# RegulatoryGenomicsGroup/chicdiff

Hardware: AMD Instinct MI355X
Metric: interactions/sec NB-GLM Wald test (higher is better)
Workload: dtype f64; 1 GPU; synthetic 2000000 interactions x 8 samples (4v4), size factors + offsets(theta=0.5) + dispersions + Wald, design ~condition; rows_per_gpu=2000000, samples=8, global_rows=2000000, parallelism=rows-sharded x1, collectives=none (single rank), ranks_in_communicator=1

## Files before the change

### chicdiff_amd/csrc/common.h

```cpp
#pragma once
#include <hip/hip_runtime.h>
#include <stdint.h>

#include "../../include/chicdiff_hip.h"
#include "fit_driver.h"
#include "fit_state.h"

namespace cd {

constexpr int kRedBlocks = 1024;

struct FitDims {
    int64_t n;
    int32_t S, p, nA, nB;
    uint64_t gmask;
};

struct FitWork {
    double *baseMean, *baseVar, *gm0, *gm1, *rough, *binit0, *binit1, *crow;
    double *dispGene, *dispFit, *dispMAP, *disp, *beta0, *beta1, *resid;
    int32_t *allZero, *geneIter, *mapIter, *outlier, *betaIter, *optimConv;
    int32_t *order;
    uint8_t *cls;
    int32_t *gridlist;
// ... 27 lines not shown
    return chunk > first_back && (uint32_t)old < stop_f;
}
__host__ __device__ inline uint32_t filler_stop_f(int percent, uint32_t chunks, uint32_t first_back) {
    if (percent >= 100) return 0xffffffffu;
    if (percent <= 0) return 0u;
    const uint32_t own = first_back < chunks ? first_back : chunks;
    return (uint32_t)(((unsigned long long)own * (unsigned)percent + 99ull) / 100ull);
}
constexpr int kRowHdr = 32;
__host__ __device__ inline int64_t row_stride(int S) {
    const int64_t bytes = kRowHdr + (int64_t)S * 12;
    return bytes <= 64 ? 64 : (bytes + 127) / 128 * 128;
}
__device__ __forceinline__ double *row_hdr(char *rowpack, int64_t r, int S) { return reinterpret_cast<double *>(rowpack + r * row_stride(S)); }

struct Opts {
    double minDisp, dispTol, kappa0, betaTol, minmu, outlierSD, dispPriorVarIn, maxDisp, trendIn[2];
    int32_t maxit, betaMaxit;
    int32_t fit_type = 0;
    int32_t spread = 1;
    int32_t min_waves = 0;
    int32_t schedule = 1;
    int32_t deal = 0;
    int32_t chunk = 0;
    int32_t classes_a = 0;
    int32_t xim_here = 0;
    int32_t prio = 0;
    int32_t fillers = -1;
    int32_t filler_stop = -1;
    int32_t trend_blocks = 0;
    int32_t trend_speculate = 1;
    int32_t mad_route = 1;
    int32_t mad_value_cap = 0;
};

constexpr int kSchedClasses = 6, kSchedBlocks = 1024;
inline void order_tiles(int64_t n, int64_t &nblk, int64_t &tile) {
    nblk = (n + 255) / 256;
    if (nblk > kSchedBlocks) nblk = kSchedBlocks;
    tile = ((n + nblk - 1) / nblk + 255) / 256 * 256;
    nblk = (n + tile - 1) / tile;
}
constexpr int kSchedClassesFine = 23, kSchedEdgesFine = 21, kSchedMinDispSlot = 17;
constexpr int kSchedSix = 3, kSchedMinDispLast = 4;
__host__ __device__ inline int sched_class(double a0, double gmin, double minDisp, int mode) {
    constexpr double edge[kSchedEdgesFine] = {0.0316, 0.0422, 0.0562, 0.0750, 0.1, 0.1334, 0.1778, 0.2371, 0.316, 0.4217, 0.5623,
                                              0.7499, 1.0, 1.3335, 1.7783, 2.3714, 3.16, 4.2170, 5.6234, 7.4989, 10.0};
    if (!(a0 > 1.5 * minDisp)) return (mode == kSchedSix || mode == kSchedMinDispLast) ? kSchedClassesFine - 1 : kSchedMinDispSlot;
    const double s = a0 * gmin;
    int f = 0;
    if (mode == kSchedSix) {
#pragma unroll
        for (int k = 4; k < kSchedEdgesFine; k += 4) f += !(s < edge[k]) ? 4 : 0;
        f += f > 0 ? 1 : 0;
    } else {
#pragma unroll
        for (int k = 0; k < kSchedEdgesFine; k++) f += !(s < edge[k]) ? 1 : 0;
    }
    return f < kSchedMinDispSlot ? f : f + 1;
}
__host__ __device__ inline int sched_classes_a(int a, int mode) {
    if (a <= 0) return 0;
    if (a <= 3) return 1 + 4 * a;
    if (a == 4) return kSchedMinDispSlot;
    if (a == 5) return (mode == kSchedSix || mode == kSchedMinDispLast) ? kSchedClassesFine - 1 : kSchedMinDispSlot;
    return kSchedClassesFine;
// ... 264 lines not shown
```

### chicdiff_amd/csrc/ctx.hip

```cpp
#include <stdarg.h>

#include <dlfcn.h>

#include "ctx.h"

char cd::g_create_err[512];

const PmcTable &cd::pmc_table(int df) {
    static PmcTable tables[4];
    static bool ready[4] = {false, false, false, false};
    static std::mutex mu;
    std::lock_guard<std::mutex> lock(mu);
    if (!ready[df]) {
        pmc_build(df, tables[df]);
        ready[df] = true;
    }
    return tables[df];
}

int cd::fail(chicdiff_hip_ctx *c, int code, const char *fmt, ...) {
    va_list ap;
    va_start(ap, fmt);
    vsnprintf(c ? c->err : g_create_err, 512, fmt, ap);
    va_end(ap);
// ... 24 lines not shown
    int32_t Opts::*tune;
    int HostOpts::*host;
    int64_t lo, hi, no_lo, no_hi;
};
static const OptionDef kOptions[] = {
    {"line_search_spread", &Opts::spread, nullptr, 0, 3, 1, 0},
    {"line_search_min_waves", &Opts::min_waves, nullptr, 0, 4, 1, 1},
    {"line_search_chunk", &Opts::chunk, nullptr, 0, 64, 1, 7},
    {"line_search_prio", &Opts::prio, nullptr, 0, 100, 1, 0},
    {"line_search_schedule", &Opts::schedule, nullptr, 0, 4, 2, 2},
    {"line_search_deal", &Opts::deal, nullptr, 0, 64, 1, 0},
    {"line_search_classes_a", &Opts::classes_a, nullptr, 0, 6, 1, 0},
    {"line_search_fillers", &Opts::fillers, nullptr, -1, 1, 1, 0},
    {"line_search_filler_stop", &Opts::filler_stop, nullptr, -1, 100, 1, 0},
    {"theta_grid_concurrency", nullptr, &HostOpts::theta_grid_concurrency, 1, 16, 1, 0},
    {"host_copy_threads", nullptr, &HostOpts::host_copy_threads, 1, 64, 1, 0},
    {"select_all_rounds", nullptr, &HostOpts::select_all_rounds, 0, 1, 1, 0},
    {"trend_one_launch_per_pass", nullptr, &HostOpts::trend_one_launch_per_pass, 0, 1, 1, 0},
    {"sharded_trend_gather", nullptr, &HostOpts::sharded_trend_gather, 0, 1, 1, 0},
    {"trend_persistent_blocks", &Opts::trend_blocks, nullptr, 0, 256, 1, 0},
    {"trend_speculate", &Opts::trend_speculate, nullptr, 0, 1, 1, 0},
    {"mad_select_route", &Opts::mad_route, nullptr, 0, 1, 1, 0},
    {"mad_value_cap", &Opts::mad_value_cap, nullptr, 0, kVbCap, 1, 0},
    {"trend_mad_in_kernel", nullptr, &HostOpts::trend_mad_in_kernel, 0, 1, 1, 0},
    {"fuse_offsets", nullptr, &HostOpts::fuse_offsets, 0, 2, 1, 0},
    {"prep_blocks", nullptr, &HostOpts::prep_blocks, 0, kRedBlocks, 1, 0},
    {"region_assemble_generic", nullptr, &HostOpts::region_assemble_generic, 0, 1, 1, 0},
    {"chicago_tables_run_merge", nullptr, &HostOpts::chicago_tables_run_merge, 0, 1, 1, 0},
    {"table_write_half_kib", nullptr, &HostOpts::table_write_half_kib, 0, 65536, 1, 3},
    {"fault_inject", nullptr, &HostOpts::fault_inject, 0, 7, 1, 0},
    {"bench_fake_world", nullptr, &HostOpts::bench_fake_world, 0, kGatherMaxWorld, 1, 0},
    {"sf_log_table", nullptr, &HostOpts::sf_log_table, 0, 1, 1, 0},
    {"wald_final_row_constant", nullptr, &HostOpts::wald_final_row_constant, 0, 1, 1, 0},
    {"local_trend_substitute", nullptr, &HostOpts::local_trend_substitute, 0, 1, 1, 0},
};

int chicdiff_hip_set_option(chicdiff_hip_ctx *c, const char *name, int64_t value) {
    if (!c || !name) return CHICDIFF_E_INVALID;
    for (const OptionDef &d : kOptions) {
        if (strcmp(name, d.name) != 0 || value < d.lo || value > d.hi || (value >= d.no_lo && value <= d.no_hi)) continue;
        if (d.host == &HostOpts::bench_fake_world && value > 1 && !getenv("CHICDIFF_BENCH_FAKE_WORLD"))
            return fail(c, CHICDIFF_E_INVALID, "set_option: bench_fake_world is a rehearsal hook of bench.py (CHICDIFF_BENCH_FAKE_WORLD unset)");
        if (d.tune) c->tune.*d.tune = (int32_t)value;
        else c->host.*d.host = (int)value;
        return CHICDIFF_OK;
    }
    return fail(c, CHICDIFF_E_INVALID, "set_option: unknown option or value (%s = %lld)", name, (long long)value);
}

int chicdiff_hip_create(chicdiff_hip_ctx **out, int32_t device) {
    if (!out) return fail(nullptr, CHICDIFF_E_INVALID, "ctx out pointer is NULL");
    *out = nullptr;
    int ndev = 0;
    hipError_t e = hipGetDeviceCount(&ndev);
    if (e != hipSuccess || ndev <= 0)
        return fail(nullptr, CHICDIFF_E_HIP, "no HIP device available (%s): the HIP path cannot run, and there is no CPU fallback",
                    e != hipSuccess ? hipGetErrorString(e) : "device count 0");
    if (device < 0 || device >= ndev) return fail(nullptr, CHICDIFF_E_INVALID, "device %d out of range [0,%d)", device, ndev);
    chicdiff_hip_ctx *c = new chicdiff_hip_ctx();
    c->device = device;
    if ((e = hipSetDevice(device)) != hipSuccess || (e = hipStreamCreateWithFlags(&c->own_stream, hipStreamNonBlocking)) != hipSuccess ||
        (e = hipHostMalloc((void **)&c->h_sc, sizeof(FitScalars))) != hipSuccess ||
        (e = hipHostMalloc((void **)&c->h_sf, sizeof(double) * (kMaxS + 1))) != hipSuccess ||
        (e = hipMalloc((void **)&c->d_sf, sizeof(double) * (kMaxS + 1 + kSelMaxWorld + 8))) != hipSuccess ||
        (e = hipMemset(c->d_sf, 0, sizeof(double) * (kMaxS + 1 + kSelMaxWorld + 8))) != hipSuccess ||
        (e = hipMalloc((void **)&c->d_logfact, sizeof(double) * kLogFactN)) != hipSuccess) {
// ... 390 lines not shown
```

### chicdiff_amd/csrc/wald_kernels.hip

```cpp
#include "common.h"
#include "devmath.h"

namespace cd {

constexpr double kLog2e = 1.4426950408889634074;

__global__ __launch_bounds__(256) void wald_prep_kernel(const int32_t *__restrict__ counts,
                                                        const double *__restrict__ nf, FitDims d, FitWork w, int sched, int64_t tile, unsigned int *hist) {
    __shared__ double s_logfact[kLogFactN];
    __shared__ LogEntry s_lt[64];
    for (int k = threadIdx.x; k < kLogFactN; k += 256) s_logfact[k] = w.logfact[k];
    log_table_to_lds(s_lt);
    const int64_t n = d.n;
    const int S = d.S;
    unsigned int mine[kSchedClasses] = {0, 0, 0, 0, 0, 0};
    const int64_t lo = tile > 0 ? (int64_t)blockIdx.x * tile : (int64_t)blockIdx.x * 256;
    const int64_t hi = tile > 0 ? (lo + tile < n ? lo + tile : n) : n;
    const int64_t step = tile > 0 ? 256 : (int64_t)gridDim.x * 256;
    for (int64_t i = lo + threadIdx.x; i < hi; i += step) {
        if (w.allZero[i]) {
            reinterpret_cast<double2 *>(w.start)[2 * i] = make_double2(NAN, 0.0);
            if (sched) {
                w.cls[i] = 255;
                w.beta0[i] = NAN;
// ... 25 lines not shown
            if ((d.gmask >> j) & 1) lB += l; else lA += l;
            if (yi > 0) {
                c += lgr_eval_t(cs, yi, s_lt) - (yi < kLogFactN ? s_logfact[yi] : lgr_eval(c1, yi));
                cst = fma((double)yi, la + tlog(nfj, s_lt), cst);
            }
        }
        lA /= d.nA;
        lB /= d.nB;
        w.binit0[i] = lA;
        w.binit1[i] = lB - lA;
        w.crow[i] = c;
        double2 *h = reinterpret_cast<double2 *>(w.start) + 2 * i;
        h[0] = make_double2(alpha, c + cst);
        h[1] = make_double2(lA, lB - lA);
    }
    if (tile > 0) order_hist_store(mine, hist);
}


__device__ __forceinline__ double optim_objective(const int32_t *y_, const double *f_, int64_t stride, int S, uint64_t gmask,
                                                  double alpha, double size, double la, double crow, double lam, double b0,
                                                  double b1) {
    double f = 0.5 * lam * (b0 * b0 + b1 * b1) - crow;
    const double E0 = exp(b0), E1 = exp(b0 + b1);
    for (int j = 0; j < S; j++) {
        const double y = (double)y_[j * stride];
        const double mu = f_[j * stride] * (((gmask >> j) & 1) ? E1 : E0);
        const double ma = alpha * mu, t = 1.0 + ma;
        f += (size + y) * flog1p_from(ma, t, rcp(t));
        if (y > 0) f -= y * (la + flog(mu));
    }
    return f;
}
__device__ __noinline__ bool optim_row(const int32_t *y_, const double *f_, int64_t stride, int S, uint64_t gmask, double alpha, double crow,
                                       double &b0, double &b1) {
    const double lam = 1e-6 / (0.69314718055994530942 * 0.69314718055994530942);
    const double bound = 30.0 * 0.69314718055994530942;
    const double size = rcp(alpha), la = flog(alpha);
    double f = optim_objective(y_, f_, stride, S, gmask, alpha, size, la, crow, lam, b0, b1);
    bool converged = false;
    for (int it = 0; it < 200 && !converged; it++) {
        double g0 = lam * b0, g1 = lam * b1, wA = 0, wB = 0;
        const double E0 = exp(b0), E1 = exp(b0 + b1);
        for (int j = 0; j < S; j++) {
            const bool g = (gmask >> j) & 1;
            const double y = (double)y_[j * stride];
            const double mu = f_[j * stride] * (g ? E1 : E0);
            const double rt = rcp(fma(alpha, mu, 1.0));
            const double sc = (y - mu) * rt, wj = mu * rt;
            g0 -= sc;
            if (g) { g1 -= sc; wB += wj; } else wA += wj;
        }
        const double m00 = wA + wB + lam, m01 = wB, m11 = wB + lam, det = m00 * m11 - m01 * m01;
        const double d0 = -(m11 * g0 - m01 * g1) / det, d1 = -(m00 * g1 - m01 * g0) / det;
        double t = 1.0;
        bool moved = false;
        for (int h = 0; h < 40; h++, t *= 0.5) {
            const double n0 = fmin(fmax(b0 + t * d0, -bound), bound), n1 = fmin(fmax(b1 + t * d1, -bound), bound);
            const double fn = optim_objective(y_, f_, stride, S, gmask, alpha, size, la, crow, lam, n0, n1);
            if (fn < f) {
                if (f - fn < 1e-13 * (fabs(f) + 1.0)) converged = true;
                b0 = n0; b1 = n1; f = fn; moved = true;
                break;
            }
        }
        if (!moved) converged = true;
    }
// ... 36 lines not shown
    if (S == 4) return load_row_sums_fixed<1>(row, s_nf, s_y, lane, gmask, iyA, iyB);
    if (S == 16) return load_row_sums_fixed<4>(row, s_nf, s_y, lane, gmask, iyA, iyB);
    if (S == 12) return load_row_sums_fixed<3>(row, s_nf, s_y, lane, gmask, iyA, iyB);
    const double *pf = reinterpret_cast<const double *>(row + kRowHdr);
    const int *py = reinterpret_cast<const int *>(row + kRowHdr + 8 * S);
    int a = 0, b = 0;
    for (int j = 0; j < S; j++) {
        const int yi = py[j];
        s_nf[j * 64 + lane] = pf[j];
        s_y[j * 64 + lane] = yi;
        if ((gmask >> j) & 1) b += yi; else a += yi;
    }
    iyA = a;
    iyB = b;
}

#ifdef CHICDIFF_DIAG
#define WDIAG(...) __VA_ARGS__
__device__ unsigned long long g_irls_cy[8], g_irls_open[2];
#else
#define WDIAG(...)
#endif
struct WaldArgs {
    const int32_t *counts;
    const double *nf;
    FitDims d;
    FitWork w;
    Opts o;
    int chunk;
    const int32_t *order;
    int spread;
};

#ifndef WALD_MINW
#define WALD_MINW 3
#endif
__global__ __launch_bounds__(256, WALD_MINW) void wald_irls_kernel(WaldArgs A) {
    extern __shared__ double smem[];
    __shared__ LogEntry s_logtab[64];
    __shared__ ExpEntry s_exptab[64];
    exp_table_to_lds(s_exptab);
    log_table_to_lds(s_logtab);
    const int lane = threadIdx.x & 63;
    const int wave = __builtin_amdgcn_readfirstlane((int)(threadIdx.x >> 6));
    const int S = A.d.S;
    const int64_t n = A.d.n;
    double *s_nf = smem + (size_t)wave * S * 96;
    int *s_y = reinterpret_cast<int *>(s_nf + S * 64);
    const uint64_t gmask = A.d.gmask;
    const Opts o = A.o;
    const double lambda = 1e-6 / (0.69314718055994530942 * 0.69314718055994530942);
    const int32_t *__restrict__ order = A.order;
    const uint32_t nTot = order ? (uint32_t)A.w.sc->ord_n : (uint32_t)n;
    unsigned long long *heads = A.w.queue + 32;
    int cur_head = blockIdx.x & 7;
    unsigned int heads_left = 0xffu;
    const uint32_t nchunks = (nTot + (uint32_t)A.chunk - 1u) / (uint32_t)A.chunk;
    const int64_t rstride = row_stride(S);

    int spread_lg = A.spread ? 1 : -1;
    while (spread_lg >= 0 && (1 << spread_lg) < S) spread_lg++;

    bool need = true, done = false, queue_empty = false;
    uint32_t chunk_pos = 0, chunk_len = 0, rest_base = 0, rest_end = 0;
    int ord_reg = 0;
    int row = -1;
    int k = 0;
    double b0 = 0, b1 = 0, alpha = 0, size = 0, crow = 0, dev_old = 0, syA = 0, syB = 0;

    WDIAG(unsigned long long cyw[8] = {0, 0, 0, 0, 0, 0, 0, 0}, wt_eval_end = 0, wr_load_end = 0, g_open_cy = 0, g_open_n = 0;)
    for (;;) {
        WDIAG(const int sec = 0; const bool sec_bulk = !queue_empty; const unsigned long long wt0 = __builtin_amdgcn_s_memtime();)
        unsigned long long needmask = __ballot(need && !done);
#pragma unroll 1
        for (int attempt = 0; needmask != 0ull && attempt < 4; attempt++) {
            WDIAG(const unsigned long long wo0 = __builtin_amdgcn_s_memtime(); const bool opened = chunk_pos >= chunk_len;)
            if (chunk_pos >= chunk_len) {
                if (rest_base >= rest_end) {
                    if (queue_empty) {
                        if (need) done = true;
                        break;
                    }
                    if (heads_left == 0u) {
                        queue_empty = true;
                        continue;
                    }
                    unsigned int kq = 0;
                    if (lane == 0) kq = (unsigned int)atomicAdd(heads + 8 * cur_head, 1ull);
                    kq = __builtin_amdgcn_readfirstlane(kq);
                    const uint32_t cq = kq * 8u + (uint32_t)cur_head;
                    if (cq >= nchunks) {
                        heads_left &= ~(1u << cur_head);
                        for (int t = 1; t <= 8; t++) {
                            const int hn = (cur_head + t) & 7;
                            if (heads_left & (1u << hn)) { cur_head = hn; break; }
                        }
                        continue;
                    }
                    rest_base = cq * (uint32_t)A.chunk;
                    rest_end = rest_base + (uint32_t)A.chunk < nTot ? rest_base + (uint32_t)A.chunk : nTot;
                }
                const uint32_t b = rest_base;
                chunk_len = rest_end - rest_base < 64u ? rest_end - rest_base : 64u;
                rest_base += chunk_len;
                chunk_pos = 0;
                ord_reg = (int)b + lane;
                if (order && (uint32_t)lane < chunk_len) ord_reg = order[b + lane];
            }
            WDIAG(if (opened && !queue_empty) { g_open_cy += __builtin_amdgcn_s_memtime() - wo0; g_open_n++; })
            const uint32_t cnt = (uint32_t)__popcll(needmask), avail = chunk_len - chunk_pos;
            const uint32_t take = cnt < avail ? cnt : avail;
            const uint32_t rank = __builtin_amdgcn_mbcnt_hi((uint32_t)(needmask >> 32), __builtin_amdgcn_mbcnt_lo((uint32_t)needmask, 0u));
            const int r = __shfl(ord_reg, (int)((chunk_pos + rank) & 63u));
            chunk_pos += take;
            WDIAG(const unsigned long long wr0 = __builtin_amdgcn_s_memtime();)
            if (need && !done && rank < take) {
                int iyA = 0, iyB = 0;
                const double2 *stp = reinterpret_cast<const double2 *>(A.w.start) + 2 * (int64_t)r;
                const double2 st0 = stp[0], st1 = stp[1];
                load_row_sums(A.w.rowpack + (int64_t)r * rstride, S, s_nf, s_y, lane, gmask, iyA, iyB);
                WDIAG(const unsigned long long wr1 = __builtin_amdgcn_s_memtime(); if (!queue_empty) { cyw[4] += wr0 - wt0; cyw[5] += wr1 - wr0; cyw[7]++; } wr_load_end = wr1;)
                if (st0.x != st0.x) {
                    A.w.beta0[r] = NAN;
                    A.w.beta1[r] = NAN;
                    A.w.betaIter[r] = 0;
                } else {
                    row = r;
                    syA = (double)iyA;
                    syB = (double)iyB;
                    alpha = st0.x;
                    size = 1.0 / alpha;
                    crow = st0.y;
                    b0 = st1.x;
                    b1 = st1.y;
                    k = 0;
                    dev_old = 0;
                    need = false;
                }
            }
            needmask = __ballot(need && !done);
            WDIAG(if (wr_load_end) { if (!queue_empty) cyw[6] += __builtin_amdgcn_s_memtime() - wr_load_end; wr_load_end = 0; })
        }
        if (__ballot(!done) == 0ull) break;
        WDIAG(const unsigned long long wt1 = __builtin_amdgcn_s_memtime();)
        const bool active = !need && !done;
        const unsigned long long actmask = __ballot(active);
        double wA = 0, wB = 0, uA = 0, uB = 0, Dl = 0, zcA = 0, zcB = 0, Dc = 0;
        const bool spread_now = queue_empty && spread_lg >= 0 && (__popcll(actmask) << spread_lg) <= 64;
        if (spread_now) {
            const int grp = lane >> spread_lg, jj = lane & ((1 << spread_lg) - 1);
            int owner = 0, nact = 0;
            for (unsigned long long m = actmask; m; m &= m - 1ull, nact++)
                if (grp == nact) owner = __ffsll((long long)m) - 1;
            const bool mine = grp < nact && jj < S;
            const double b0o = __shfl(b0, owner), b1o = __shfl(b1, owner), alo = __shfl(alpha, owner), szo = __shfl(size, owner);
            const double etaAo = b0o, etaBo = b0o + b1o;
            const double E0 = texp(etaAo, s_exptab), E1 = texp(etaBo, s_exptab);
            const double nfj = mine ? s_nf[jj * 64 + owner] : 1.0;
            const double y = mine ? (double)s_y[jj * 64 + owner] : 0.0;
            const bool g = (gmask >> jj) & 1;
            const double raw = nfj * (g ? E1 : E0);
            const bool floored = raw < o.minmu;
            const double mu = floored ? o.minmu : raw;
            const double ma = alo * mu;
            const double t1 = 1.0 + ma;
            const double rt = rcp(t1);
            const double wj = mu * rt;
            const double yr = y * rt;
            const double sy = szo + y;
            const double L = tlog1p_from(ma, t1, rt, s_logtab);
            double de = 0.0;
            if (floored) de = (tlog(o.minmu, s_logtab) - tlog(nfj, s_logtab)) - (g ? etaBo : etaAo);
            const int fl = floored ? 1 : 0;
            const int base = grp << spread_lg;
            for (int j0 = 0; j0 < S; j0 += 4) {
                double q_wj[4], q_yr[4], q_sy[4], q_L[4], q_de[4], q_y[4];
                int q_fl[4];
#pragma unroll
                for (int t = 0; t < 4; t++) {
                    const int src = base + (j0 + t < S ? j0 + t : j0);
                    q_wj[t] = __shfl(wj, src);
                    q_yr[t] = __shfl(yr, src);
                    q_sy[t] = __shfl(sy, src);
                    q_L[t] = __shfl(L, src);
                    q_fl[t] = __shfl(fl, src);
                    q_de[t] = __shfl(de, src);
                    q_y[t] = __shfl(y, src);
                }
#pragma unroll
                for (int t = 0; t < 4; t++) {
                    if (j0 + t >= S) continue;
                    const bool gj = (gmask >> (j0 + t)) & 1;
                    const double gB = gj ? 1.0 : 0.0, gA = gj ? 0.0 : 1.0;
                    wA = fma(q_wj[t], gA, wA);
                    wB = fma(q_wj[t], gB, wB);
                    uA = fma(q_yr[t], gA, uA);
                    uB = fma(q_yr[t], gB, uB);
                    Dl = fma(q_sy[t], q_L[t], Dl);
                    if (q_fl[t]) {
                        if (gj) zcB = fma(q_wj[t], q_de[t], zcB); else zcA = fma(q_wj[t], q_de[t], zcA);
                        Dc = fma(-q_y[t], q_de[t], Dc);
                    }
                }
            }
            const int src = (active ? __popcll(actmask & ((1ull << lane) - 1ull)) : 0) << spread_lg;
            wA = __shfl(wA, src);
            wB = __shfl(wB, src);
            uA = __shfl(uA, src);
            uB = __shfl(uB, src);
            Dl = __shfl(Dl, src);
            zcA = __shfl(zcA, src);
            zcB = __shfl(zcB, src);
            Dc = __shfl(Dc, src);
        }
        if (active) {

            const double etaA = b0, etaB = b0 + b1;
            double E0 = 0, E1 = 0;
            if (!spread_now) {
                E0 = texp(etaA, s_exptab);
                E1 = texp(etaB, s_exptab);
            }
            for (int j = 0; j < (spread_now ? 0 : S); j++) {
                const double nfj = s_nf[j * 64 + lane];
                const double y = (double)s_y[j * 64 + lane];
                const bool g = (gmask >> j) & 1;
                const double raw = nfj * (g ? E1 : E0);
                const bool floored = raw < o.minmu;
                const double mu = floored ? o.minmu : raw;
                const double ma = alpha * mu;
                const double t1 = 1.0 + ma;
                const double rt = rcp(t1);
                const double wj = mu * rt;
                const double gB = g ? 1.0 : 0.0, gA = g ? 0.0 : 1.0;
                const double yr = y * rt;
                wA = fma(wj, gA, wA);
                wB = fma(wj, gB, wB);
                uA = fma(yr, gA, uA);
                uB = fma(yr, gB, uB);
                Dl = fma(size + y, tlog1p_from(ma, t1, rt, s_logtab), Dl);
                if (floored) {
                    const double de = (tlog(o.minmu, s_logtab) - tlog(nfj, s_logtab)) - (g ? etaB : etaA);
                    if (g) zcB = fma(wj, de, zcB); else zcA = fma(wj, de, zcA);
                    Dc = fma(-y, de, Dc);
                }
            }
            WDIAG(const unsigned long long wt2 = __builtin_amdgcn_s_memtime(); if (sec_bulk) { cyw[sec + 0] += wt1 - wt0; cyw[sec + 1] += wt2 - wt1; cyw[sec + 3]++; wt_eval_end = wt2; })
            const double zA = fma(etaA - 1.0, wA, uA) + zcA, zB = fma(etaB - 1.0, wB, uB) + zcB;
            const double D = (Dl - fma(etaA, syA, etaB * syB)) + Dc;
            bool stop = false;
            int iter_out = k;
            if (k >= 1) {
                const double dev = 2.0 * (D - crow);
                const double diff = fabs(dev - dev_old), scale = fabs(dev) + 0.1;
                if (!(diff == diff) || !(scale == scale) || (isinf(diff) && isinf(scale))) {
                    stop = true;
                    iter_out = o.betaMaxit;
                } else if (k >= 2 && diff < o.betaTol * scale) {
                    stop = true;
                } else if (k >= o.betaMaxit) {
                    stop = true;
                }
                dev_old = dev;
            }
            if (!stop) {
                const double m00 = wA + wB + lambda, m01 = wB, m11 = wB + lambda;
                const double r0 = zA + zB, r1 = zB;
                const double idet = rcp(fma(m00, m11, -(m01 * m01)));
                b0 = fma(m11, r0, -(m01 * r1)) * idet;
                b1 = fma(m00, r1, -(m01 * r0)) * idet;
                k++;
                if (fabs(b0) > 30.0 || fabs(b1) > 30.0) {
                    stop = true;
                    iter_out = o.betaMaxit;
                }
            }
            if (stop) {
                if (iter_out >= o.betaMaxit) {
                    b0 = A.w.binit0[row];
                    b1 = A.w.binit1[row];
                    A.w.optimConv[row] = optim_row(s_y + lane, s_nf + lane, 64, S, gmask, alpha, A.w.crow[row], b0, b1) ? 1 : 0;
                }
                A.w.beta0[row] = b0;
                A.w.beta1[row] = b1;
                A.w.betaIter[row] = iter_out;
                need = true;
            }
        }
        WDIAG(if (wt_eval_end) { cyw[sec + 2] += __builtin_amdgcn_s_memtime() - wt_eval_end; wt_eval_end = 0; })
    }
    WDIAG(if (lane == 0) { for (int q = 0; q < 8; q++) atomicAdd(&g_irls_cy[q], cyw[q]); atomicAdd(&g_irls_open[0], g_open_cy); atomicAdd(&g_irls_open[1], g_open_n); })
}


__device__ __forceinline__ int trim_lo(int n) {
    const double tr = n <= 3 ? 1.0 / 3 : (n <= 23 ? 1.0 / 4 : 1.0 / 8);
    return (int)floor(n * tr);
}
__device__ __forceinline__ double trim_scale(int n) { return n <= 3 ? 2.04 : (n <= 23 ? 1.86 : 1.51); }

__device__ __forceinline__ double cell_trimmed_mean(const double *s_q, int T, int tid, int S, uint64_t gmask, int c,
                                                    int nc, int lo, bool sq, double cm) {
    double sum = 0;
    if (lo == 1) {
        int imin = -1, imax = -1;
        double vmin = INFINITY, vmax = -INFINITY;
        for (int j = 0; j < S; j++) {
            if ((int)((gmask >> j) & 1) != c) continue;
            double vj = s_q[j * T + tid];
            if (sq) vj = (vj - cm) * (vj - cm);
            if (vj < vmin) { vmin = vj; imin = j; }
            if (vj >= vmax) { vmax = vj; imax = j; }
        }
        for (int j = 0; j < S; j++) {
            if ((int)((gmask >> j) & 1) != c || j == imin || j == imax) continue;
            double vj = s_q[j * T + tid];
            if (sq) vj = (vj - cm) * (vj - cm);
            sum += vj;
        }
        return sum / (nc - 2);
    }
    for (int j = 0; j < S; j++) {
// ... 243 lines not shown
        for (int b = threadIdx.x; b < kRedBlocks; b += 256) acc += w.partials[(size_t)b * 3 + k];
        red[threadIdx.x] = acc;
        __syncthreads();
        for (int s = 128; s > 0; s >>= 1) {
            if ((int)threadIdx.x < s) red[threadIdx.x] += red[threadIdx.x + s];
            __syncthreads();
        }
        if (threadIdx.x == 0) sums[k] = red[0];
        __syncthreads();
    }
    if (threadIdx.x == 0) {
        sums[3] = w.sc->failed == 3 ? 1.0 : 0.0;
        sums[4] = w.sc->neg_counts ? 1.0 : 0.0;
        sums[5] = w.sc->sel_overflow ? 1.0 : 0.0;
        sums[6] = (carry && *carry) ? 1.0 : 0.0;
        sums[7] = 0.0;
    }
    if (sf_dev && (int)threadIdx.x < S) w.sc->final_sf[threadIdx.x] = sf_dev[threadIdx.x];
}

static bool irls_schedule(const FitDims &d, const Opts &o) { return o.schedule && d.n > 131072; }
void launch_wald_prep(const int32_t *counts, const double *nf, FitDims d, FitWork w, Opts o, hipStream_t st) {
    o.schedule = irls_schedule(d, o) ? o.schedule : 0;
    int64_t nblk, tile;
    order_tiles(d.n, nblk, tile);
    if (o.schedule && tile == 256) {
        wald_prep_kernel<<<(unsigned)nblk, 256, 0, st>>>(counts, nf, d, w, o.schedule, tile, reinterpret_cast<unsigned int *>(w.hist));
        launch_order_build(d, w, 0, true, st);
        return;
    }
    wald_prep_kernel<<<1536, 256, 0, st>>>(counts, nf, d, w, o.schedule, 0, nullptr);
    if (o.schedule) launch_order_build(d, w, 0, false, st);
}
void launch_wald_irls(const int32_t *counts, const double *nf, FitDims d, FitWork w, Opts o, hipStream_t st) {
    WaldArgs A{counts, nf, d, w, o, 64, irls_schedule(d, o) ? w.order : nullptr, o.spread};
    const size_t lds_per_wave = (size_t)d.S * 64 * 12;
    int threads = 256;
    while (threads > 64 && lds_per_wave * (threads / 64) > 40 * 1024) threads >>= 1;
    const size_t lds = lds_per_wave * (threads / 64);
    int64_t blocks = ((d.n + 63) / 64 + threads / 64 - 1) / (threads / 64);
    int64_t per_cu = (int64_t)(160 * 1024 / lds) < 8 ? (int64_t)(160 * 1024 / lds) : 8;
    const int64_t by_regs = 4 * WALD_MINW / (threads / 64);
    if (per_cu > by_regs) per_cu = by_regs;
    if (blocks > 256 * per_cu) blocks = 256 * per_cu;
    if (blocks < 1) blocks = 1;
    const int64_t per_wave = d.n / (blocks * (threads / 64));
    A.chunk = per_wave >= 256 ? 128 : 64;
#ifdef CHICDIFF_DIAG
    const bool stamps = getenv("CHICDIFF_IRLS_STAMPS") != nullptr;
    if (stamps) {
        unsigned long long z[8] = {0, 0, 0, 0, 0, 0, 0, 0};
        (void)hipMemcpyToSymbol(HIP_SYMBOL(g_irls_cy), z, sizeof z);
        (void)hipMemcpyToSymbol(HIP_SYMBOL(g_irls_open), z, 16);
    }
#endif
    wald_irls_kernel<<<(unsigned)blocks, threads, lds, st>>>(A);
#ifdef CHICDIFF_DIAG
    if (stamps) {
        (void)hipStreamSynchronize(st);
        unsigned long long h[8];
        (void)hipMemcpyFromSymbol(h, HIP_SYMBOL(g_irls_cy), sizeof h);
        {
            const double t = h[3] ? (double)h[3] : 1.0, r = h[7] ? (double)h[7] : 1.0;
            printf("  IRLS ticks while the queue has rows (lane 0 of every wave): %.0f per wave; s_memtime cycles per tick: refill %.0f, evaluate %.0f, solve + state %.0f\n",
                   t / (double)(blocks * (threads / 64)), h[0] / t, h[1] / t, h[2] / t);
            unsigned long long ho[2];
            (void)hipMemcpyFromSymbol(ho, HIP_SYMBOL(g_irls_open), sizeof ho);
            printf("    pieces of the schedule opened: %.1f per wave, %.0f cycles each\n", (double)ho[1] / (double)(blocks * (threads / 64)), ho[1] ? (double)ho[0] / (double)ho[1] : 0.0);
            printf("    inside a refill that lane 0 took part in (%.0f per wave): tick start -> loads issued %.0f, loads issued -> row in LDS %.0f, -> end of the attempt %.0f cycles\n",
                   r / (double)(blocks * (threads / 64)), h[4] / r, h[5] / r, h[6] / r);
        }
    }
#endif
}
void launch_wald_final(const int32_t *counts, const double *nf, FitDims d, FitWork w, Opts o, int row_constant,
                       const chicdiff_nbglm_out &out, hipStream_t st) {
    const int threads = d.S <= 16 ? 256 : 64;
    wald_final_kernel<<<kRedBlocks, threads, (size_t)d.S * threads * sizeof(double), st>>>(counts, nf, d, w, o, row_constant, out);
}
void launch_wald_intercept(const int32_t *counts, const double *nf, FitDims d, FitWork w, Opts,
                           const chicdiff_nbglm_out &out, hipStream_t st) {
    wald_intercept_kernel<<<kRedBlocks, 256, 0, st>>>(counts, nf, d, w, out);
}
void launch_dev_sum_finish(FitDims d, FitWork w, const int32_t *carry, const double *sf_dev, hipStream_t st) {
    dev_sum_kernel<<<1, 256, 0, st>>>(w, carry, sf_dev, d.S);
}

}
```

Measured before the change: 619.6 million interactions/s.

## Defer optim fallback rows into per-lane list, template IRLS kernel on wave occupancy

IRLS rows that need the optim fallback no longer run it inline. They are chained into a per-lane deferred list stored through optimConv, and lanes drain that list together after the main loop, or early while the queue is non-empty when MINW<4. optim_row is now force-inlined, and the kernel is templated on the launch_bounds minimum waves, selectable as 3 (default) or 4 through a new option. The aim is to keep the rare fallback path from causing divergence and register pressure in the hot loop. In exchange the loop is more complex and the rows have to be reloaded after an early drain.

Result: no change. 624.8 million interactions/s, median of 6 (+0.8%).

```diff
diff --git a/chicdiff_amd/csrc/common.h b/chicdiff_amd/csrc/common.h
--- a/chicdiff_amd/csrc/common.h
+++ b/chicdiff_amd/csrc/common.h
@@ -83,6 +83,7 @@
     int32_t trend_speculate = 1;
     int32_t mad_route = 1;
     int32_t mad_value_cap = 0;
+    int32_t irls_waves = 0;
 };
 
 constexpr int kSchedClasses = 6, kSchedBlocks = 1024;
diff --git a/chicdiff_amd/csrc/ctx.hip b/chicdiff_amd/csrc/ctx.hip
--- a/chicdiff_amd/csrc/ctx.hip
+++ b/chicdiff_amd/csrc/ctx.hip
@@ -80,6 +80,7 @@
     {"bench_fake_world", nullptr, &HostOpts::bench_fake_world, 0, kGatherMaxWorld, 1, 0},
     {"sf_log_table", nullptr, &HostOpts::sf_log_table, 0, 1, 1, 0},
     {"wald_final_row_constant", nullptr, &HostOpts::wald_final_row_constant, 0, 1, 1, 0},
+    {"wald_irls_waves", &Opts::irls_waves, nullptr, 0, 4, 1, 2},
     {"local_trend_substitute", nullptr, &HostOpts::local_trend_substitute, 0, 1, 1, 0},
 };
 
diff --git a/chicdiff_amd/csrc/wald_kernels.hip b/chicdiff_amd/csrc/wald_kernels.hip
--- a/chicdiff_amd/csrc/wald_kernels.hip
+++ b/chicdiff_amd/csrc/wald_kernels.hip
@@ -81,7 +81,7 @@
     }
     return f;
 }
-__device__ __noinline__ bool optim_row(const int32_t *y_, const double *f_, int64_t stride, int S, uint64_t gmask, double alpha, double crow,
+__device__ __forceinline__ bool optim_row(const int32_t *y_, const double *f_, int64_t stride, int S, uint64_t gmask, double alpha, double crow,
                                        double &b0, double &b1) {
     const double lam = 1e-6 / (0.69314718055994530942 * 0.69314718055994530942);
     const double bound = 30.0 * 0.69314718055994530942;
@@ -184,15 +184,14 @@
     int spread;
 };
 
-#ifndef WALD_MINW
-#define WALD_MINW 3
-#endif
-__global__ __launch_bounds__(256, WALD_MINW) void wald_irls_kernel(WaldArgs A) {
+template <int MINW>
+__global__ __launch_bounds__(256, MINW) void wald_irls_kernel(WaldArgs A) {
     extern __shared__ double smem[];
     __shared__ LogEntry s_logtab[64];
     __shared__ ExpEntry s_exptab[64];
     exp_table_to_lds(s_exptab);
     log_table_to_lds(s_logtab);
+    constexpr bool kEarlyDrain = MINW < 4;
     const int lane = threadIdx.x & 63;
     const int wave = __builtin_amdgcn_readfirstlane((int)(threadIdx.x >> 6));
     const int S = A.d.S;
@@ -219,227 +218,269 @@
     int row = -1;
     int k = 0;
     double b0 = 0, b1 = 0, alpha = 0, size = 0, crow = 0, dev_old = 0, syA = 0, syB = 0;
+    int defer = -1;
 
     WDIAG(unsigned long long cyw[8] = {0, 0, 0, 0, 0, 0, 0, 0}, wt_eval_end = 0, wr_load_end = 0, g_open_cy = 0, g_open_n = 0;)
     for (;;) {
-        WDIAG(const int sec = 0; const bool sec_bulk = !queue_empty; const unsigned long long wt0 = __builtin_amdgcn_s_memtime();)
-        unsigned long long needmask = __ballot(need && !done);
+        bool early = false;
+        for (;;) {
+            WDIAG(const int sec = 0; const bool sec_bulk = !queue_empty; const unsigned long long wt0 = __builtin_amdgcn_s_memtime();)
+            unsigned long long needmask = __ballot(need && !done);
 #pragma unroll 1
-        for (int attempt = 0; needmask != 0ull && attempt < 4; attempt++) {
-            WDIAG(const unsigned long long wo0 = __builtin_amdgcn_s_memtime(); const bool opened = chunk_pos >= chunk_len;)
-            if (chunk_pos >= chunk_len) {
-                if (rest_base >= rest_end) {
-                    if (queue_empty) {
-                        if (need) done = true;
-                        break;
-                    }
-                    if (heads_left == 0u) {
-                        queue_empty = true;
-                        continue;
-                    }
-                    unsigned int kq = 0;
-                    if (lane == 0) kq = (unsigned int)atomicAdd(heads + 8 * cur_head, 1ull);
-                    kq = __builtin_amdgcn_readfirstlane(kq);
-                    const uint32_t cq = kq * 8u + (uint32_t)cur_head;
-                    if (cq >= nchunks) {
-                        heads_left &= ~(1u << cur_head);
-                        for (int t = 1; t <= 8; t++) {
-                            const int hn = (cur_head + t) & 7;
-                            if (heads_left & (1u << hn)) { cur_head = hn; break; }
+            for (int attempt = 0; needmask != 0ull && attempt < 4; attempt++) {
+                WDIAG(const unsigned long long wo0 = __builtin_amdgcn_s_memtime(); const bool opened = chunk_pos >= chunk_len;)
+                if (chunk_pos >= chunk_len) {
+                    if (rest_base >= rest_end) {
+                        if (queue_empty) {
+                            if (need) done = true;
+                            break;
                         }
-                        continue;
-                    }
-                    rest_base = cq * (uint32_t)A.chunk;
-                    rest_end = rest_base + (uint32_t)A.chunk < nTot ? rest_base + (uint32_t)A.chunk : nTot;
-                }
-                const uint32_t b = rest_base;
-                chunk_len = rest_end - rest_base < 64u ? rest_end - rest_base : 64u;
-                rest_base += chunk_len;
-                chunk_pos = 0;
-                ord_reg = (int)b + lane;
-                if (order && (uint32_t)lane < chunk_len) ord_reg = order[b + lane];
-            }
-            WDIAG(if (opened && !queue_empty) { g_open_cy += __builtin_amdgcn_s_memtime() - wo0; g_open_n++; })
-            const uint32_t cnt = (uint32_t)__popcll(needmask), avail = chunk_len - chunk_pos;
-            const uint32_t take = cnt < avail ? cnt : avail;
-            const uint32_t rank = __builtin_amdgcn_mbcnt_hi((uint32_t)(needmask >> 32), __builtin_amdgcn_mbcnt_lo((uint32_t)needmask, 0u));
-            const int r = __shfl(ord_reg, (int)((chunk_pos + rank) & 63u));
-            chunk_pos += take;
-            WDIAG(const unsigned long long wr0 = __builtin_amdgcn_s_memtime();)
-            if (need && !done && rank < take) {
-                int iyA = 0, iyB = 0;
-                const double2 *stp = reinterpret_cast<const double2 *>(A.w.start) + 2 * (int64_t)r;
-                const double2 st0 = stp[0], st1 = stp[1];
-                load_row_sums(A.w.rowpack + (int64_t)r * rstride, S, s_nf, s_y, lane, gmask, iyA, iyB);
-                WDIAG(const unsigned long long wr1 = __builtin_amdgcn_s_memtime(); if (!queue_empty) { cyw[4] += wr0 - wt0; cyw[5] += wr1 - wr0; cyw[7]++; } wr_load_end = wr1;)
-                if (st0.x != st0.x) {
-                    A.w.beta0[r] = NAN;
-                    A.w.beta1[r] = NAN;
-                    A.w.betaIter[r] = 0;
-                } else {
-                    row = r;
-                    syA = (double)iyA;
-                    syB = (double)iyB;
-                    alpha = st0.x;
-                    size = 1.0 / alpha;
-                    crow = st0.y;
-                    b0 = st1.x;
-                    b1 = st1.y;
-                    k = 0;
-                    dev_old = 0;
-                    need = false;
-                }
-            }
-            needmask = __ballot(need && !done);
-            WDIAG(if (wr_load_end) { if (!queue_empty) cyw[6] += __builtin_amdgcn_s_memtime() - wr_load_end; wr_load_end = 0; })
-        }
-        if (__ballot(!done) == 0ull) break;
-        WDIAG(const unsigned long long wt1 = __builtin_amdgcn_s_memtime();)
-        const bool active = !need && !done;
-        const unsigned long long actmask = __ballot(active);
-        double wA = 0, wB = 0, uA = 0, uB = 0, Dl = 0, zcA = 0, zcB = 0, Dc = 0;
-        const bool spread_now = queue_empty && spread_lg >= 0 && (__popcll(actmask) << spread_lg) <= 64;
-        if (spread_now) {
-            const int grp = lane >> spread_lg, jj = lane & ((1 << spread_lg) - 1);
-            int owner = 0, nact = 0;
-            for (unsigned long long m = actmask; m; m &= m - 1ull, nact++)
-                if (grp == nact) owner = __ffsll((long long)m) - 1;
-            const bool mine = grp < nact && jj < S;
-            const double b0o = __shfl(b0, owner), b1o = __shfl(b1, owner), alo = __shfl(alpha, owner), szo = __shfl(size, owner);
-            const double etaAo = b0o, etaBo = b0o + b1o;
-            const double E0 = texp(etaAo, s_exptab), E1 = texp(etaBo, s_exptab);
-            const double nfj = mine ? s_nf[jj * 64 + owner] : 1.0;
-            const double y = mine ? (double)s_y[jj * 64 + owner] : 0.0;
-            const bool g = (gmask >> jj) & 1;
-            const double raw = nfj * (g ? E1 : E0);
-            const bool floored = raw < o.minmu;
-            const double mu = floored ? o.minmu : raw;
-            const double ma = alo * mu;
-            const double t1 = 1.0 + ma;
-            const double rt = rcp(t1);
-            const double wj = mu * rt;
-            const double yr = y * rt;
-            const double sy = szo + y;
-            const double L = tlog1p_from(ma, t1, rt, s_logtab);
-            double de = 0.0;
-            if (floored) de = (tlog(o.minmu, s_logtab) - tlog(nfj, s_logtab)) - (g ? etaBo : etaAo);
-            const int fl = floored ? 1 : 0;
-            const int base = grp << spread_lg;
-            for (int j0 = 0; j0 < S; j0 += 4) {
-                double q_wj[4], q_yr[4], q_sy[4], q_L[4], q_de[4], q_y[4];
-                int q_fl[4];
-#pragma unroll
-                for (int t = 0; t < 4; t++) {
-                    const int src = base + (j0 + t < S ? j0 + t : j0);
-                    q_wj[t] = __shfl(wj, src);
-                    q_yr[t] = __shfl(yr, src);
-                    q_sy[t] = __shfl(sy, src);
-                    q_L[t] = __shfl(L, src);
-                    q_fl[t] = __shfl(fl, src);
-                    q_de[t] = __shfl(de, src);
-                    q_y[t] = __shfl(y, src);
-                }
-#pragma unroll
-                for (int t = 0; t < 4; t++) {
-                    if (j0 + t >= S) continue;
-                    const bool gj = (gmask >> (j0 + t)) & 1;
-                    const double gB = gj ? 1.0 : 0.0, gA = gj ? 0.0 : 1.0;
-                    wA = fma(q_wj[t], gA, wA);
-                    wB = fma(q_wj[t], gB, wB);
-                    uA = fma(q_yr[t], gA, uA);
-                    uB = fma(q_yr[t], gB, uB);
-                    Dl = fma(q_sy[t], q_L[t], Dl);
-                    if (q_fl[t]) {
-                        if (gj) zcB = fma(q_wj[t], q_de[t], zcB); else zcA = fma(q_wj[t], q_de[t], zcA);
-                        Dc = fma(-q_y[t], q_de[t], Dc);
-                    }
-                }
-            }
-            const int src = (active ? __popcll(actmask & ((1ull << lane) - 1ull)) : 0) << spread_lg;
-            wA = __shfl(wA, src);
-            wB = __shfl(wB, src);
-            uA = __shfl(uA, src);
-            uB = __shfl(uB, src);
-            Dl = __shfl(Dl, src);
-            zcA = __shfl(zcA, src);
-            zcB = __shfl(zcB, src);
-            Dc = __shfl(Dc, src);
-        }
-        if (active) {
-
-            const double etaA = b0, etaB = b0 + b1;
-            double E0 = 0, E1 = 0;
-            if (!spread_now) {
-                E0 = texp(etaA, s_exptab);
-                E1 = texp(etaB, s_exptab);
-            }
-            for (int j = 0; j < (spread_now ? 0 : S); j++) {
-                const double nfj = s_nf[j * 64 + lane];
-                const double y = (double)s_y[j * 64 + lane];
-                const bool g = (gmask >> j) & 1;
+                        if (heads_left == 0u) {
+                            queue_empty = true;
+                            continue;
+                        }
+                        unsigned int kq = 0;
+                        if (lane == 0) kq = (unsigned int)atomicAdd(heads + 8 * cur_head, 1ull);
+                        kq = __builtin_amdgcn_readfirstlane(kq);
+                        const uint32_t cq = kq * 8u + (uint32_t)cur_head;
+                        if (cq >= nchunks) {
+                            heads_left &= ~(1u << cur_head);
+                            for (int t = 1; t <= 8; t++) {
+                                const int hn = (cur_head + t) & 7;
+                                if (heads_left & (1u << hn)) { cur_head = hn; break; }
+                            }
+                            continue;
+                        }
+                        rest_base = cq * (uint32_t)A.chunk;
+                        rest_end = rest_base + (uint32_t)A.chunk < nTot ? rest_base + (uint32_t)A.chunk : nTot;
+                    }
+                    const uint32_t b = rest_base;
+                    chunk_len = rest_end - rest_base < 64u ? rest_end - rest_base : 64u;
+                    rest_base += chunk_len;
+                    chunk_pos = 0;
+                    ord_reg = (int)b + lane;
+                    if (order && (uint32_t)lane < chunk_len) ord_reg = order[b + lane];
+                }
+                WDIAG(if (opened && !queue_empty) { g_open_cy += __builtin_amdgcn_s_memtime() - wo0; g_open_n++; })
+                const uint32_t cnt = (uint32_t)__popcll(needmask), avail = chunk_len - chunk_pos;
+                const uint32_t take = cnt < avail ? cnt : avail;
+                const uint32_t rank = __builtin_amdgcn_mbcnt_hi((uint32_t)(needmask >> 32), __builtin_amdgcn_mbcnt_lo((uint32_t)needmask, 0u));
+                const int r = __shfl(ord_reg, (int)((chunk_pos + rank) & 63u));
+                chunk_pos += take;
+                WDIAG(const unsigned long long wr0 = __builtin_amdgcn_s_memtime();)
+                if (need && !done && rank < take) {
+                    int iyA = 0, iyB = 0;
+                    const double2 *stp = reinterpret_cast<const double2 *>(A.w.start) + 2 * (int64_t)r;
+                    const double2 st0 = stp[0], st1 = stp[1];
+                    load_row_sums(A.w.rowpack + (int64_t)r * rstride, S, s_nf, s_y, lane, gmask, iyA, iyB);
+                    WDIAG(const unsigned long long wr1 = __builtin_amdgcn_s_memtime(); if (!queue_empty) { cyw[4] += wr0 - wt0; cyw[5] += wr1 - wr0; cyw[7]++; } wr_load_end = wr1;)
+                    if (st0.x != st0.x) {
+                        A.w.beta0[r] = NAN;
+                        A.w.beta1[r] = NAN;
+                        A.w.betaIter[r] = 0;
+                    } else {
+                        row = r;
+                        syA = (double)iyA;
+                        syB = (double)iyB;
+                        alpha = st0.x;
+                        size = 1.0 / alpha;
+                        crow = st0.y;
+                        b0 = st1.x;
+                        b1 = st1.y;
+                        k = 0;
+                        dev_old = 0;
+                        need = false;
+                    }
+                }
+                needmask = __ballot(need && !done);
+                WDIAG(if (wr_load_end) { if (!queue_empty) cyw[6] += __builtin_amdgcn_s_memtime() - wr_load_end; wr_load_end = 0; })
+            }
+            if (__ballot(!done) == 0ull) break;
+            WDIAG(const unsigned long long wt1 = __builtin_amdgcn_s_memtime();)
+            const bool active = !need && !done;
+            const unsigned long long actmask = __ballot(active);
+            double wA = 0, wB = 0, uA = 0, uB = 0, Dl = 0, zcA = 0, zcB = 0, Dc = 0;
+            const bool spread_now = queue_empty && spread_lg >= 0 && (__popcll(actmask) << spread_lg) <= 64;
+            if (spread_now) {
+                const int grp = lane >> spread_lg, jj = lane & ((1 << spread_lg) - 1);
+                int owner = 0, nact = 0;
+                for (unsigned long long m = actmask; m; m &= m - 1ull, nact++)
+                    if (grp == nact) owner = __ffsll((long long)m) - 1;
+                const bool mine = grp < nact && jj < S;
+                const double b0o = __shfl(b0, owner), b1o = __shfl(b1, owner), alo = __shfl(alpha, owner), szo = __shfl(size, owner);
+                const double etaAo = b0o, etaBo = b0o + b1o;
+                const double E0 = texp(etaAo, s_exptab), E1 = texp(etaBo, s_exptab);
+                const double nfj = mine ? s_nf[jj * 64 + owner] : 1.0;
+                const double y = mine ? (double)s_y[jj * 64 + owner] : 0.0;
+                const bool g = (gmask >> jj) & 1;
                 const double raw = nfj * (g ? E1 : E0);
                 const bool floored = raw < o.minmu;
                 const double mu = floored ? o.minmu : raw;
-                const double ma = alpha * mu;
+                const double ma = alo * mu;
                 const double t1 = 1.0 + ma;
                 const double rt = rcp(t1);
                 const double wj = mu * rt;
-                const double gB = g ? 1.0 : 0.0, gA = g ? 0.0 : 1.0;
                 const double yr = y * rt;
-                wA = fma(wj, gA, wA);
-                wB = fma(wj, gB, wB);
-                uA = fma(yr, gA, uA);
-                uB = fma(yr, gB, uB);
-                Dl = fma(size + y, tlog1p_from(ma, t1, rt, s_logtab), Dl);
-                if (floored) {
-                    const double de = (tlog(o.minmu, s_logtab) - tlog(nfj, s_logtab)) - (g ? etaB : etaA);
-                    if (g) zcB = fma(wj, de, zcB); else zcA = fma(wj, de, zcA);
-                    Dc = fma(-y, de, Dc);
-                }
-            }
-            WDIAG(const unsigned long long wt2 = __builtin_amdgcn_s_memtime(); if (sec_bulk) { cyw[sec + 0] += wt1 - wt0; cyw[sec + 1] += wt2 - wt1; cyw[sec + 3]++; wt_eval_end = wt2; })
-            const double zA = fma(etaA - 1.0, wA, uA) + zcA, zB = fma(etaB - 1.0, wB, uB) + zcB;
-            const double D = (Dl - fma(etaA, syA, etaB * syB)) + Dc;
-            bool stop = false;
-            int iter_out = k;
-            if (k >= 1) {
-                const double dev = 2.0 * (D - crow);
-                const double diff = fabs(dev - dev_old), scale = fabs(dev) + 0.1;
-                if (!(diff == diff) || !(scale == scale) || (isinf(diff) && isinf(scale))) {
-                    stop = true;
-                    iter_out = o.betaMaxit;
-                } else if (k >= 2 && diff < o.betaTol * scale) {
-                    stop = true;
-                } else if (k >= o.betaMaxit) {
-                    stop = true;
-                }
-                dev_old = dev;
-            }
-            if (!stop) {
-                const double m00 = wA + wB + lambda, m01 = wB, m11 = wB + lambda;
-                const double r0 = zA + zB, r1 = zB;
-                const double idet = rcp(fma(m00, m11, -(m01 * m01)));
-                b0 = fma(m11, r0, -(m01 * r1)) * idet;
-                b1 = fma(m00, r1, -(m01 * r0)) * idet;
-                k++;
-                if (fabs(b0) > 30.0 || fabs(b1) > 30.0) {
-                    stop = true;
-                    iter_out = o.betaMaxit;
-                }
-            }
-            if (stop) {
-                if (iter_out >= o.betaMaxit) {
-                    b0 = A.w.binit0[row];
-                    b1 = A.w.binit1[row];
-                    A.w.optimConv[row] = optim_row(s_y + lane, s_nf + lane, 64, S, gmask, alpha, A.w.crow[row], b0, b1) ? 1 : 0;
-                }
-                A.w.beta0[row] = b0;
-                A.w.beta1[row] = b1;
-                A.w.betaIter[row] = iter_out;
-                need = true;
-            }
-        }
-        WDIAG(if (wt_eval_end) { cyw[sec + 2] += __builtin_amdgcn_s_memtime() - wt_eval_end; wt_eval_end = 0; })
+                const double sy = szo + y;
+                const double L = tlog1p_from(ma, t1, rt, s_logtab);
+                double de = 0.0;
+                if (floored) de = (tlog(o.minmu, s_logtab) - tlog(nfj, s_logtab)) - (g ? etaBo : etaAo);
+                const int fl = floored ? 1 : 0;
+                const int base = grp << spread_lg;
+                constexpr int FQ = MINW >= 4 ? 2 : 4;
+                for (int j0 = 0; j0 < S; j0 += FQ) {
+                    double q_wj[FQ], q_yr[FQ], q_sy[FQ], q_L[FQ], q_de[FQ], q_y[FQ];
+                    int q_fl[FQ];
+#pragma unroll
+                    for (int t = 0; t < FQ; t++) {
+                        const int src = base + (j0 + t < S ? j0 + t : j0);
+                        q_wj[t] = __shfl(wj, src);
+                        q_yr[t] = __shfl(yr, src);
+                        q_sy[t] = __shfl(sy, src);
+                        q_L[t] = __shfl(L, src);
+                        q_fl[t] = __shfl(fl, src);
+                        q_de[t] = __shfl(de, src);
+                        q_y[t] = __shfl(y, src);
+                    }
+#pragma unroll
+                    for (int t = 0; t < FQ; t++) {
+                        if (j0 + t >= S) continue;
+                        const bool gj = (gmask >> (j0 + t)) & 1;
+                        const double gB = gj ? 1.0 : 0.0, gA = gj ? 0.0 : 1.0;
+                        wA = fma(q_wj[t], gA, wA);
+                        wB = fma(q_wj[t], gB, wB);
+                        uA = fma(q_yr[t], gA, uA);
+                        uB = fma(q_yr[t], gB, uB);
+                        Dl = fma(q_sy[t], q_L[t], Dl);
+                        if (q_fl[t]) {
+                            if (gj) zcB = fma(q_wj[t], q_de[t], zcB); else zcA = fma(q_wj[t], q_de[t], zcA);
+                            Dc = fma(-q_y[t], q_de[t], Dc);
+                        }
+                    }
+                }
+                const int src = (active ? __popcll(actmask & ((1ull << lane) - 1ull)) : 0) << spread_lg;
+                wA = __shfl(wA, src);
+                wB = __shfl(wB, src);
+                uA = __shfl(uA, src);
+                uB = __shfl(uB, src);
+                Dl = __shfl(Dl, src);
+                zcA = __shfl(zcA, src);
+                zcB = __shfl(zcB, src);
+                Dc = __shfl(Dc, src);
+            }
+            int fb = -1;
+            if (active) {
+
+                const double etaA = b0, etaB = b0 + b1;
+                double E0 = 0, E1 = 0;
+                if (!spread_now) {
+                    E0 = texp(etaA, s_exptab);
+                    E1 = texp(etaB, s_exptab);
+                }
+                for (int j = 0; j < (spread_now ? 0 : S); j++) {
+                    const double nfj = s_nf[j * 64 + lane];
+                    const double y = (double)s_y[j * 64 + lane];
+                    const bool g = (gmask >> j) & 1;
+                    const double raw = nfj * (g ? E1 : E0);
+                    const bool floored = raw < o.minmu;
+                    const double mu = floored ? o.minmu : raw;
+                    const double ma = alpha * mu;
+                    const double t1 = 1.0 + ma;
+                    const double rt = rcp(t1);
+                    const double wj = mu * rt;
+                    const double gB = g ? 1.0 : 0.0, gA = g ? 0.0 : 1.0;
+                    const double yr = y * rt;
+                    wA = fma(wj, gA, wA);
+                    wB = fma(wj, gB, wB);
+                    uA = fma(yr, gA, uA);
+                    uB = fma(yr, gB, uB);
+                    Dl = fma(size + y, tlog1p_from(ma, t1, rt, s_logtab), Dl);
+                    if (floored) {
+                        const double de = (tlog(o.minmu, s_logtab) - tlog(nfj, s_logtab)) - (g ? etaB : etaA);
+                        if (g) zcB = fma(wj, de, zcB); else zcA = fma(wj, de, zcA);
+                        Dc = fma(-y, de, Dc);
+                    }
+                }
+                WDIAG(const unsigned long long wt2 = __builtin_amdgcn_s_memtime(); if (sec_bulk) { cyw[sec + 0] += wt1 - wt0; cyw[sec + 1] += wt2 - wt1; cyw[sec + 3]++; wt_eval_end = wt2; })
+                const double zA = fma(etaA - 1.0, wA, uA) + zcA, zB = fma(etaB - 1.0, wB, uB) + zcB;
+                const double D = (Dl - fma(etaA, syA, etaB * syB)) + Dc;
+                bool stop = false;
+                int iter_out = k;
+                if (k >= 1) {
+                    const double dev = 2.0 * (D - crow);
+                    const double diff = fabs(dev - dev_old), scale = fabs(dev) + 0.1;
+                    if (!(diff == diff) || !(scale == scale) || (isinf(diff) && isinf(scale))) {
+                        stop = true;
+                        iter_out = o.betaMaxit;
+                    } else if (k >= 2 && diff < o.betaTol * scale) {
+                        stop = true;
+                    } else if (k >= o.betaMaxit) {
+                        stop = true;
+                    }
+                    dev_old = dev;
+                }
+                if (!stop) {
+                    const double m00 = wA + wB + lambda, m01 = wB, m11 = wB + lambda;
+                    const double r0 = zA + zB, r1 = zB;
+                    const double idet = rcp(fma(m00, m11, -(m01 * m01)));
+                    b0 = fma(m11, r0, -(m01 * r1)) * idet;
+                    b1 = fma(m00, r1, -(m01 * r0)) * idet;
+                    k++;
+                    if (fabs(b0) > 30.0 || fabs(b1) > 30.0) {
+                        stop = true;
+                        iter_out = o.betaMaxit;
+                    }
+                }
+                if (stop) {
+                    if (iter_out >= o.betaMaxit) {
+                        fb = row;
+                    } else {
+                        A.w.beta0[row] = b0;
+                        A.w.beta1[row] = b1;
+                    }
+                    A.w.betaIter[row] = iter_out;
+                    need = true;
+                }
+            }
+            WDIAG(if (wt_eval_end) { cyw[sec + 2] += __builtin_amdgcn_s_memtime() - wt_eval_end; wt_eval_end = 0; })
+            unsigned long long fbmask = __ballot(fb >= 0);
+            if (__builtin_expect_with_probability(fbmask != 0ull, 0, 0.999999)) {
+                unsigned long long freemask = __ballot(defer < 0 && fb < 0);
+                fbmask = __ballot(fb >= 0 && defer >= 0);
+                for (; fbmask != 0ull && freemask != 0ull; fbmask &= fbmask - 1ull, freemask &= freemask - 1ull) {
+                    const int from = __ffsll((long long)fbmask) - 1, to = __ffsll((long long)freemask) - 1;
+                    const int r = __shfl(fb, from);
+                    if (lane == to) fb = r;
+                    if (lane == from) fb = -1;
+                }
+                if (fb >= 0) {
+                    A.w.optimConv[fb] = defer;
+                    defer = fb;
+                }
+                if (kEarlyDrain && !queue_empty) {
+                    early = true;
+                    break;
+                }
+            }
+        }
+        if (__builtin_expect_with_probability(__ballot(defer >= 0) != 0ull, 0, 0.999999))
+        while (__ballot(defer >= 0) != 0ull) {
+            if (defer >= 0) {
+                const int r = defer;
+                defer = A.w.optimConv[r];
+                int iyA = 0, iyB = 0;
+                load_row_sums(A.w.rowpack + (int64_t)r * rstride, S, s_nf, s_y, lane, gmask, iyA, iyB);
+                double o0 = A.w.binit0[r], o1 = A.w.binit1[r];
+                A.w.optimConv[r] = optim_row(s_y + lane, s_nf + lane, 64, S, gmask, A.w.start[4 * (int64_t)r], A.w.crow[r], o0, o1) ? 1 : 0;
+                A.w.beta0[r] = o0;
+                A.w.beta1[r] = o1;
+            }
+        }
+        if (!early) break;
+        if (!need && !done) {
+            int iyA = 0, iyB = 0;
+            load_row_sums(A.w.rowpack + (int64_t)row * rstride, S, s_nf, s_y, lane, gmask, iyA, iyB);
+        }
     }
     WDIAG(if (lane == 0) { for (int q = 0; q < 8; q++) atomicAdd(&g_irls_cy[q], cyw[q]); atomicAdd(&g_irls_open[0], g_open_cy); atomicAdd(&g_irls_open[1], g_open_n); })
 }
@@ -749,6 +790,7 @@
     wald_prep_kernel<<<1536, 256, 0, st>>>(counts, nf, d, w, o.schedule, 0, nullptr);
     if (o.schedule) launch_order_build(d, w, 0, false, st);
 }
+static int irls_waves(const Opts &o) { return o.irls_waves ? o.irls_waves : 3; }
 void launch_wald_irls(const int32_t *counts, const double *nf, FitDims d, FitWork w, Opts o, hipStream_t st) {
     WaldArgs A{counts, nf, d, w, o, 64, irls_schedule(d, o) ? w.order : nullptr, o.spread};
     const size_t lds_per_wave = (size_t)d.S * 64 * 12;
@@ -757,7 +799,8 @@
     const size_t lds = lds_per_wave * (threads / 64);
     int64_t blocks = ((d.n + 63) / 64 + threads / 64 - 1) / (threads / 64);
     int64_t per_cu = (int64_t)(160 * 1024 / lds) < 8 ? (int64_t)(160 * 1024 / lds) : 8;
-    const int64_t by_regs = 4 * WALD_MINW / (threads / 64);
+    const int minw = irls_waves(o);
+    const int64_t by_regs = 4 * minw / (threads / 64);
     if (per_cu > by_regs) per_cu = by_regs;
     if (blocks > 256 * per_cu) blocks = 256 * per_cu;
     if (blocks < 1) blocks = 1;
@@ -771,7 +814,8 @@
         (void)hipMemcpyToSymbol(HIP_SYMBOL(g_irls_open), z, 16);
     }
 #endif
-    wald_irls_kernel<<<(unsigned)blocks, threads, lds, st>>>(A);
+    if (minw == 4) wald_irls_kernel<4><<<(unsigned)blocks, threads, lds, st>>>(A);
+    else wald_irls_kernel<3><<<(unsigned)blocks, threads, lds, st>>>(A);
 #ifdef CHICDIFF_DIAG
     if (stamps) {
         (void)hipStreamSynchronize(st);
```
